# nickirk/pymes

Hardware: AMD Instinct MI355X
Metric: ccsd_iteration_time (lower is better)
Workload: dtype f64

## Files before the change

pymes_amd/csrc/kernels.hip:

```cpp
#include <hip/hip_runtime.h>
#include <type_traits>

#include <algorithm>
#include <atomic>
#include <chrono>
#include <cmath>
#include <cstdio>
#include <cstdlib>
#include <cstring>
#include <mutex>
#include <stdexcept>
#include <string>
#include <vector>

#include "device_api.h"
#include "diis_small.h"

#define HIP_CHECK(expr)                                                                   \
    do {                                                                                  \
        hipError_t err__ = (expr);                                                        \
        if (err__ != hipSuccess)                                                          \
            throw std::runtime_error(std::string("HIP error: ") + hipGetErrorString(err__) + \
                                     " at " __FILE__ ":" + std::to_string(__LINE__));     \
    } while (0)
// ... 1784 lines not shown
    const double* __restrict__ Ba = B + (long)(no + a) * n + no;
    const double* __restrict__ Bb = B + (long)(no + b) * n + no;
    const int t = threadIdx.x, lane = t & 63, w = t >> 6;
    const int wc = (w >> 1) * 16, wd = (w & 1) * 16, l15 = lane & 15, l4 = lane >> 4;
    const int lx = t & 31, lk = t >> 5;
    v4d X = {0.0, 0.0, 0.0, 0.0}, Y = {0.0, 0.0, 0.0, 0.0};
    for (int q0 = 0; q0 < naux; q0 += kFacK) {
#pragma unroll
        for (int h = 0; h < 2; ++h) {
            const int k = lk + 8 * h, q = q0 + k;
            const long qo = (long)q * nn;
            const bool cok = q < naux && c0 + lx < nv, dok = q < naux && d0 + lx < nv;
            sAc[k][lx] = cok ? Ba[qo + c0 + lx] : 0.0;
            sBc[k][lx] = cok ? Bb[qo + c0 + lx] : 0.0;
            sAd[k][lx] = dok ? Ba[qo + d0 + lx] : 0.0;
            sBd[k][lx] = dok ? Bb[qo + d0 + lx] : 0.0;
        }
        __syncthreads();
#pragma unroll
        for (int kk = 0; kk < kFacK; kk += 4) {
            const int k = kk + l4;
            X = __builtin_amdgcn_mfma_f64_16x16x4f64(sAc[k][wc + l15], sBd[k][wd + l15], X, 0, 0, 0);
            Y = __builtin_amdgcn_mfma_f64_16x16x4f64(sBc[k][wc + l15], sAd[k][wd + l15], Y, 0, 0, 0);
        }
        __syncthreads();
    }
    const int d = d0 + wd + l15;
#pragma unroll
    for (int i = 0; i < 4; ++i) {
        const int c = c0 + wc + l4 + 4 * i;
        if (c < nv && d < nv && c >= d) {
            Vp[row * npp + (long)c * (c + 1) / 2 + d] = X[i] + Y[i];
            if (c > d) Vm[row * npm + (long)c * (c - 1) / 2 + d] = (a > b) ? X[i] - Y[i] : 0.0;
        }
    }
}

__global__ void ladder_dress_tfrag_kernel(const double* __restrict__ t1, double* __restrict__ tf, int no, int nv, int nk, long total) {
    const long e = blockIdx.x * (long)blockDim.x + threadIdx.x;
    if (e >= total) return;
    const int L = (int)(e & 63), kk = (int)((e >> 6) % nk), tile = (int)((e >> 6) / nk);
    const int a = 16 * tile + (L & 15), k = 4 * kk + (L >> 4);
    tf[e] = (a < nv && k < no) ? -t1[(long)a * no + k] : 0.0;
}

template <int NK>
__global__ void __launch_bounds__(64) ladder_dress_kernel(const double* __restrict__ V, const double* __restrict__ Pk,
                                                          const double* __restrict__ tf, double* __restrict__ W, int no,
                                                          int nv, long ld, long row0, long row1, double sgn, long ntp) {
    constexpr int TP = 16 * 16 + 16;
    __shared__ double turn[16 * TP];
    const int lane = threadIdx.x, g = lane >> 4, c = lane & 15;
    const long idx = blockIdx.x >> 3;
    const long cdb = (blockIdx.x & 7) + 8 * (idx / ntp), tp = idx % ntp;
    if (cdb * 16 >= ld) return;
    int ta_, tb_;
    unrank_pair(tp, ta_, tb_);
    const int a0 = ta_ * 16, b0 = tb_ * 16;
    const long tri0 = (long)a0 * (a0 + 1) / 2;
    if (tri0 + (long)15 * a0 + 120 + b0 + 15 < row0 || tri0 + b0 >= row1) return;
    double ta[NK], tb[NK];
#pragma unroll
    for (int kk = 0; kk < NK; ++kk) {
        ta[kk] = tf[((long)ta_ * NK + kk) * 64 + lane];
        tb[kk] = tf[((long)tb_ * NK + kk) * 64 + lane];
    }
    typedef unsigned v2u __attribute__((ext_vector_type(2)));
    constexpr unsigned kOff = 0x80000000u;
    const long col = cdb * 16 + c;
    const unsigned lo = (unsigned)(8 * ((long)g * ld + col));
    const unsigned lo_last = (unsigned)(8 * ((long)(min(4 * (NK - 1) + g, no - 1) - 4 * (NK - 1)) * ld + col));
    const unsigned ldb = (unsigned)(8 * ld);
    const __amdgpu_buffer_rsrc_t rPa = __builtin_amdgcn_make_buffer_rsrc(const_cast<double*>(Pk + (long)a0 * no * ld), 0, kOff, 0x00020000);
    const __amdgpu_buffer_rsrc_t rPb = __builtin_amdgcn_make_buffer_rsrc(const_cast<double*>(Pk + (long)b0 * no * ld), 0, kOff, 0x00020000);
    const __amdgpu_buffer_rsrc_t rV = __builtin_amdgcn_make_buffer_rsrc(const_cast<double*>(V + (tri0 - row0) * ld), 0, kOff, 0x00020000);
    const __amdgpu_buffer_rsrc_t rW = __builtin_amdgcn_make_buffer_rsrc(W + (tri0 - row0) * ld, 0, kOff, 0x00020000);
    unsigned vo[4];
#pragma unroll
    for (int r = 0; r < 4; ++r) {
        const long a = a0 + g + 4 * r;
        vo[r] = a < nv ? (unsigned)(8 * ((a * (a + 1) / 2 - tri0) * ld + col)) : kOff;
    }
    auto row_off = [&](int r, int x) {
        const int a = a0 + g + 4 * r;
        const long row = (long)a * (a + 1) / 2 + x;
        return (x <= a && row >= row0 && row < row1) ? vo[r] : kOff;
    };
    constexpr int PA = 1, NBP = 2 * (PA + 1), VA = 3, NBV = 2 * (VA + 1);
    double pf[NBP][NK], vin[NBV][4];
    auto fetch_p = [&](int n) {
        const int x0 = n < 16 ? a0 : b0, i = n < 16 ? n : n - 16;
        const unsigned so = (unsigned)(min(x0 + i, nv - 1) - x0) * (unsigned)no * ldb;
        const __amdgpu_buffer_rsrc_t rs = n < 16 ? rPa : rPb;
#pragma unroll
        for (int kk = 0; kk < NK - 1; ++kk)
            pf[n % NBP][kk] = __builtin_bit_cast(double, __builtin_amdgcn_raw_buffer_load_b64(rs, lo, so + 4u * kk * ldb, 0));
        pf[n % NBP][NK - 1] = __builtin_bit_cast(double, __builtin_amdgcn_raw_buffer_load_b64(rs, lo_last, so + 4u * (NK - 1) * ldb, 0));
    };
    auto fetch_v = [&](int n) {
        const int x = b0 + n - 16;
#pragma unroll
        for (int r = 0; r < 4; ++r)
            vin[n % NBV][r] = __builtin_bit_cast(double, __builtin_amdgcn_raw_buffer_load_b64(rV, row_off(r, x), (unsigned)x * ldb, 2));
    };
#pragma unroll
    for (int n = 0; n < 2 * PA; ++n) fetch_p(n);
#pragma unroll
    for (int p = 0; p < 8; ++p) {
        const int n0 = 2 * p, n1 = n0 + 1;
        fetch_p(n0 + 2 * PA);
        fetch_p(n1 + 2 * PA);
        if (n0 + 2 * VA >= 16) { fetch_v(n0 + 2 * VA); fetch_v(n1 + 2 * VA); }
        v4d acc0 = {0.0, 0.0, 0.0, 0.0}, acc1 = {0.0, 0.0, 0.0, 0.0};
#pragma unroll
        for (int kk = 0; kk < NK; ++kk) {
            acc0 = __builtin_amdgcn_mfma_f64_16x16x4f64(tb[kk], pf[n0 % NBP][kk], acc0, 0, 0, 0);
            acc1 = __builtin_amdgcn_mfma_f64_16x16x4f64(tb[kk], pf[n1 % NBP][kk], acc1, 0, 0, 0);
        }
#pragma unroll
        for (int rb = 0; rb < 4; ++rb) {
            turn[n0 * TP + (g + 4 * rb) * 16 + c] = acc0[rb];
            turn[n1 * TP + (g + 4 * rb) * 16 + c] = acc1[rb];
        }
    }
    __builtin_amdgcn_fence(__ATOMIC_SEQ_CST, "wavefront");
    __builtin_amdgcn_wave_barrier();
    const double s2 = sgn > 0.0 ? -1.0 : 1.0;
#pragma unroll
    for (int p = 0; p < 8; ++p) {
        const int b = 2 * p, n0 = 16 + b, n1 = n0 + 1;
        if (n0 + 2 * PA < 32) { fetch_p(n0 + 2 * PA); fetch_p(n1 + 2 * PA); }
        if (n0 + 2 * VA < 32) { fetch_v(n0 + 2 * VA); fetch_v(n1 + 2 * VA); }
        v4d acc0, acc1;
#pragma unroll
        for (int r = 0; r < 4; ++r) {
            acc0[r] = fma(s2, turn[(g + 4 * r) * TP + b * 16 + c], vin[n0 % NBV][r]);
            acc1[r] = fma(s2, turn[(g + 4 * r) * TP + (b + 1) * 16 + c], vin[n1 % NBV][r]);
        }
#pragma unroll
        for (int kk = 0; kk < NK; ++kk) {
            acc0 = __builtin_amdgcn_mfma_f64_16x16x4f64(ta[kk], pf[n0 % NBP][kk], acc0, 0, 0, 0);
            acc1 = __builtin_amdgcn_mfma_f64_16x16x4f64(ta[kk], pf[n1 % NBP][kk], acc1, 0, 0, 0);
        }
#pragma unroll
        for (int h = 0; h < 2; ++h) {
            const int bb = b0 + b + h;
#pragma unroll
            for (int r = 0; r < 4; ++r) {
                const double val = (sgn > 0.0 && a0 + g + 4 * r == bb) ? 0.0 : (double)(h ? acc1[r] : acc0[r]);
                __builtin_amdgcn_raw_buffer_store_b64(__builtin_bit_cast(v2u, val), rW, row_off(r, bb), (unsigned)bb * ldb, 2);
            }
        }
    }
}

struct PackTK {
    const double* T; const double* t1; double* Sp; double* Am;
    long ldp, ldm, rp0;
    int no, nv, flags;
};
__device__ __forceinline__ void ladder_pack_T_body(const PackTK& k, const unsigned vb) {
    const double* __restrict__ T = k.T;
    const double* __restrict__ t1 = k.t1;
    double* __restrict__ Sp = k.Sp;
    double* __restrict__ Am = k.Am;
    const int no = k.no, nv = k.nv, flags = k.flags;
    const long ldp = k.ldp, ldm = k.ldm;
    const long row = k.rp0 + vb;
    int c, d;
    unrank_pair(row, c, d);
    const bool row_half = flags & dev::PACK_ROW_HALF, prow = flags & dev::PACK_AM_PROWS,
               col_half = flags & dev::PACK_COL_HALF, pcol = flags & dev::PACK_AM_PCOLS;
    const long o2 = (long)no * no;
    const double* __restrict__ T1 = T ? T + ((long)c * nv + d) * o2 : nullptr;
    const double* __restrict__ T2 = T ? T + ((long)d * nv + c) * o2 : nullptr;
    const double fr = (c == d && row_half) ? 0.25 : 0.5;
    const long mrow = prow ? row : (long)c * (c - 1) / 2 + d;
    const bool has_m = prow || c > d;
    if (threadIdx.x == 0) {
        const long opp = (long)no * (no + 1) / 2, mcols = pcol ? opp : opp - no;
        if (ldp > opp) Sp[row * ldp + opp] = 0.0;
        if (has_m && ldm > mcols) Am[mrow * ldm + mcols] = 0.0;
    }
    for (int e = threadIdx.x; e < o2; e += blockDim.x) {
        const int i = e / no, j = e - i * no;
        if (i < j) continue;
        double x1 = 0.0, x2 = 0.0;
        if (T) { x1 = T1[e]; x2 = T2[e]; }
        if (t1) {
            x1 += t1[(long)c * no + i] * t1[(long)d * no + j];
            x2 += t1[(long)d * no + i] * t1[(long)c * no + j];
        }
        Sp[row * ldp + (long)i * (i + 1) / 2 + j] = ((i == j && col_half) ? 0.5 * fr : fr) * (x1 + x2);
        if (has_m && (pcol || i > j)) {
            const long mcol = pcol ? (long)i * (i + 1) / 2 + j : (long)i * (i - 1) / 2 + j;
            Am[mrow * ldm + mcol] = (c > d && i > j) ? 0.5 * (x1 - x2) : 0.0;
        }
    }
}
__global__ void ladder_pack_T_kernel(const PackTK k) { ladder_pack_T_body(k, blockIdx.x); }

struct UnpackK {
    const double* L; double* R;
    double beta;
    long total;
    int no, nv;
};
__device__ __forceinline__ void ladder_unpack_body(const UnpackK& k, const unsigned vb, const unsigned vgrid) {
    const double* __restrict__ L = k.L;
    double* __restrict__ R = k.R;
    const double beta = k.beta;
    const int no = k.no, nv = k.nv;
    const long total = k.total;
    const long opp = (long)no * (no + 1) / 2, ld = (long)no * no;
    for (long idx = vb * (long)blockDim.x + threadIdx.x; idx < total; idx += (long)vgrid * blockDim.x) {
        long r = idx;
        const int j = (int)(r % no); r /= no;
        const int i = (int)(r % no); r /= no;
        const int b = (int)(r % nv);
        const int a = (int)(r / nv);
        const int ah = max(a, b), al = min(a, b), ih = max(i, j), il = min(i, j);
        const double* __restrict__ row = L + ((long)ah * (ah + 1) / 2 + al) * ld;
        double v = row[(long)ih * (ih + 1) / 2 + il];
        if (a != b && i != j) {
            const double x = row[opp + (long)ih * (ih - 1) / 2 + il];
            v += ((a > b) == (i > j)) ? x : -x;
        }
        R[idx] = (beta != 0.0) ? beta * R[idx] + v : v;
    }
}
__global__ void ladder_unpack_kernel(const UnpackK k) { ladder_unpack_body(k, blockIdx.x, gridDim.x); }

struct RingOpK {
    const double* Wd; const double* Ud; double* M; double* N1;
    double a1, a2;
    int no, nv;
};
__device__ __forceinline__ void ring_operands_body(const RingOpK& q, const unsigned vb) {
    const double* __restrict__ Wd = q.Wd;
    const double* __restrict__ Ud = q.Ud;
    double* __restrict__ M = q.M;
    double* __restrict__ N1 = q.N1;
    const double a1 = q.a1, a2 = q.a2;
    const int no = q.no, nv = q.nv;
    extern __shared__ double tile[];
    constexpr int CT = 32;
    const int k = vb / nv, b = vb - k * nv;
    const long ov = (long)no * nv;
    const double* __restrict__ wd = Wd + ((long)k * nv + b) * ((long)nv * no);
    const double* __restrict__ ud = Ud + ((long)k * nv + b) * ((long)no * nv);
    const long col = (long)b * no;
    for (int c0 = 0; c0 < nv; c0 += CT) {
        const int nc = min(CT, nv - c0);
        for (int e = threadIdx.x; e < no * CT; e += blockDim.x) {
            const int j = e / CT, cc = e - j * CT;
            if (cc < nc) tile[j * (CT + 1) + cc] = ud[(long)j * nv + c0 + cc];
        }
        __syncthreads();
        for (int e = threadIdx.x; e < nc * no; e += blockDim.x) {
            const int cc = e / no, j = e - cc * no;
            const double u = tile[j * (CT + 1) + cc];
            const double w = wd[(long)(c0 + cc) * no + j];
            const long off = ((long)(c0 + cc) * no + k) * ov + col + j;
            N1[off] = -u;
            M[off] = a1 * w - a2 * u;
        }
        __syncthreads();
    }
}
__global__ void __launch_bounds__(256) ring_operands_kernel(const RingOpK q) { ring_operands_body(q, blockIdx.x); }

struct LayoutsK {
    const double* T; double* Td; double* Tx; double* Ttd;
    double ca, cb;
    int no, nv;
};
template <bool RESIDUAL>
__device__ __forceinline__ void t2_layouts_body(const LayoutsK& k, const unsigned vb) {
    const double* __restrict__ T = k.T;
    double* __restrict__ Td = k.Td;
    double* __restrict__ Tx = k.Tx;
    double* __restrict__ Ttd = k.Ttd;
    const int no = k.no, nv = k.nv;
    const double ca = k.ca, cb = k.cb;
    extern __shared__ double tile[];
    const int a = vb / nv, b = vb - a * nv;
    const long o2 = (long)no * no, ov = (long)no * nv;
    const double* __restrict__ Tab = T + ((long)a * nv + b) * o2;
    const double* __restrict__ Tba = T + ((long)b * nv + a) * o2;
    const long base = (long)a * no * ov + (long)b * no;
    for (int e = threadIdx.x; e < o2; e += blockDim.x) {
        const int i = e / no, j = e - i * no;
        const double x = Tab[e];
        tile[i * (no + 1) + j] = x;
        const long off = base + (long)i * ov + j;
        if (Td) Td[off] = x;
        Ttd[off] = RESIDUAL ? 2.0 * x - Tba[e] : ca * x + cb * Tba[e];
    }
    __syncthreads();
    for (int e = threadIdx.x; e < o2; e += blockDim.x) {
        const int j = e / no, i = e - j * no;
        Tx[base + (long)j * ov + i] = tile[i * (no + 1) + j];
    }
}
template <bool RESIDUAL>
__global__ void __launch_bounds__(256) t2_layouts_kernel(const LayoutsK k) { t2_layouts_body<RESIDUAL>(k, blockIdx.x); }
// ... 2567 lines not shown
    };
    for (int i0 = 0; i0 < mx; i0 += 16)
        for (int j0 = 0; j0 < ny; j0 += 4) {
            const int mm = std::min(16, mx - i0), nn = std::min(4, ny - j0);
            int NN = 4;
            double* tile = tiles + 64 * done.size();
            if (mm <= 4) gram_tile_n<4>(X + i0, mm, Y + j0, nn, (long)len, vec, nblk, ws, tile, st, NN);
            else if (mm <= 8) gram_tile_n<8>(X + i0, mm, Y + j0, nn, (long)len, vec, nblk, ws, tile, st, NN);
            else if (mm <= 12) gram_tile_n<12>(X + i0, mm, Y + j0, nn, (long)len, vec, nblk, ws, tile, st, NN);
            else gram_tile_n<16>(X + i0, mm, Y + j0, nn, (long)len, vec, nblk, ws, tile, st, NN);
            done.push_back({i0, mm, j0, nn, NN});
            if ((int)done.size() == kGramTiles) flush();
        }
    flush();
}

void lincomb_multi(int m, int n, const double* const* x, const double* c, const double* beta, double* const* y, int64_t len,
                   stream_t s) {
    if (n <= 0 || len <= 0) return;
    if (m < 0 || m > 64 || n > 64) throw std::runtime_error("lincomb_multi: at most 64 inputs and 64 outputs per call");
    if (m > 16 || n > 4)
        for (int j = 0; j < n; ++j)
            for (int i = 0; i < m; ++i)
                if (y[j] == x[i]) throw std::runtime_error("lincomb_multi: an output may alias an input only for m <= 16, n <= 4");
    hipStream_t st = (hipStream_t)s;
    bool vec = true;
    for (int i = 0; i < m; ++i) vec = vec && aligned16(x[i]);
    for (int j = 0; j < n; ++j) vec = vec && aligned16(y[j]);
    double one[4] = {1.0, 1.0, 1.0, 1.0}, b0[4];
    for (int j0 = 0; j0 < n; j0 += 4) {
        const int nn = std::min(4, n - j0);
        for (int j = 0; j < nn; ++j) b0[j] = beta ? beta[j0 + j] : 0.0;
        if (m == 0) {
            const double* none[1] = {y[j0]};
            const double zero[4] = {0.0, 0.0, 0.0, 0.0};
            lincomb_multi_tile_n<4>(none, 1, zero, 4, b0, y + j0, nn, (long)len, vec, st);
            continue;
        }
        for (int i0 = 0; i0 < m; i0 += 16) {
            const int mm = std::min(16, m - i0);
            const double* bb = i0 == 0 ? b0 : one;
            const double* cc = c + (long)i0 * n + j0;
            if (mm <= 4) lincomb_multi_tile_n<4>(x + i0, mm, cc, n, bb, y + j0, nn, (long)len, vec, st);
            else if (mm <= 8) lincomb_multi_tile_n<8>(x + i0, mm, cc, n, bb, y + j0, nn, (long)len, vec, st);
            else if (mm <= 12) lincomb_multi_tile_n<12>(x + i0, mm, cc, n, bb, y + j0, nn, (long)len, vec, st);
            else lincomb_multi_tile_n<16>(x + i0, mm, cc, n, bb, y + j0, nn, (long)len, vec, st);
        }
    }
}

void cmul(const double* mr, const double* mi, const double* xr, const double* xi, double* yr, double* yi, int64_t n, stream_t s) {
    if (n <= 0) return;
    PYMES_LAUNCH(cmul_kernel, dim3(grid_for(n)), dim3(256), 0, (hipStream_t)s, mr, mi, xr, xi, yr, yi, (long)n);
    HIP_CHECK(hipGetLastError());
}

void exchange_split(const double* u, double* us, double* w, double* dg, int no, int nv, stream_t s) {
    const long total = (long)nv * nv * no * no;
    if (!total) return;
    PYMES_LAUNCH(exchange_split_kernel, dim3(grid_for(total, 256, 256 * 64)), dim3(256), 0, (hipStream_t)s, u, us, w, dg, no, nv,
                       total);
    HIP_CHECK(hipGetLastError());
}
void sgn_ij_add(double* D, const double* R, int no, int nv, stream_t s) {
    const long total = (long)nv * nv * no * no;
    if (!total) return;
    PYMES_LAUNCH(sgn_ij_add_kernel, dim3(grid_for(total, 256, 256 * 64)), dim3(256), 0, (hipStream_t)s, D, R, no, total);
    HIP_CHECK(hipGetLastError());
}
int64_t eom_diag_ws_doubles(int no, int nv) { return EomDiagWs(no, nv).total; }
void eom_diagonals(const double* V, const double* T, const double* dai, const double* iaai, const double* iaia, const double* ijij,
                   const double* abab, double* d1, double* d2, int no, int nv, double* ws, stream_t s) {
    hipStream_t st = (hipStream_t)s;
    const EomDiagWs w(no, nv);
    const long total = (long)nv * nv * no * no;
    if (w.total > 0x7fffffffL) throw std::runtime_error("eom_diagonals: problem too large for one grid");
    PYMES_LAUNCH(eom_diag_sums_kernel, dim3((unsigned)w.total), dim3(256), 0, st, V, T, ws, no, nv);
    HIP_CHECK(hipGetLastError());
    PYMES_LAUNCH(eom_diag_singles_kernel, dim3((unsigned)(((long)nv * no + 255) / 256)), dim3(256), 0, st, ws, dai, iaai, iaia,
                       d1, no, nv);
    HIP_CHECK(hipGetLastError());
    PYMES_LAUNCH(eom_diag_doubles_kernel, dim3(grid_for(total, 256, 256 * 64)), dim3(256), 0, st, V, T, ws, dai, iaai, iaia, ijij,
                       abab, d2, no, nv, total);
    HIP_CHECK(hipGetLastError());
}
void cshift_inv(const double* d, double zr, double zi, double hr, double hi, double shift, double* mr, double* mi, int64_t n,
                stream_t s) {
    if (n <= 0) return;
    PYMES_LAUNCH(cshift_inv_kernel, dim3(grid_for(n)), dim3(256), 0, (hipStream_t)s, d, zr, zi, hr, hi, shift, mr, mi, (long)n);
    HIP_CHECK(hipGetLastError());
}

void tau_build(double* tau, const double* t2, const double* t1, int no, int nv, stream_t s) {
    const long total = (long)nv * nv * no * no;
    if (!total) return;
    const TauK k{tau, t2, t1, total, no, nv};
    const double cost = 16.0 * (double)total / 4.0e6;
    if (phase_open((hipStream_t)s) && phase_small(cost)) {
        PhaseRec& t = phase_push(PK_TAU, 0, grid_for(total), 0, cost, k);
        phase_reads(t, {prange(t2, total), prange(t1, (long)no * nv)});
        phase_writes(t, {prange(tau, total)});
        return;
    }
    PYMES_LAUNCH(tau_kernel, dim3(grid_for(total)), dim3(256), 0, (hipStream_t)s, k);
    HIP_CHECK(hipGetLastError());
}

void ladder_pack_V(const double* V, double* Vp, double* Vm, int nr, int nc, int64_t rp0, int64_t rp1, stream_t s, int64_t ldvp,
                   int64_t ldvm) {
    if (rp1 <= rp0) return;
    const long npp = ldvp ? (long)ldvp : (long)nc * (nc + 1) / 2, npm = ldvm ? (long)ldvm : (long)nc * (nc - 1) / 2;
    const int nt = (nc + 31) / 32;
    const long ntp = (long)nt * (nt + 1) / 2;
    const long nblk = (rp1 - rp0) * ntp;
    if (nblk > 0x7fffffffL) throw std::runtime_error("ladder_pack_V: grid too large");
    PYMES_LAUNCH(ladder_pack_V_kernel, dim3((unsigned)nblk), dim3(256), 0, (hipStream_t)s, V, Vp, Vm, nr, nc,
                       (long)rp0, nt, ntp, npp, npm);
    HIP_CHECK(hipGetLastError());
}

void ladder_pack_V_factors(const double* B, double* Vp, double* Vm, int naux, int n, int no, int64_t rp0, int64_t rp1,
                           stream_t s, int64_t ldvp, int64_t ldvm) {
    if (rp1 <= rp0) return;
    const int nv = n - no;
    if (naux < 1 || no < 0 || nv < 1 || rp0 < 0 || rp1 > (int64_t)nv * (nv + 1) / 2)
        throw std::runtime_error("ladder_pack_V_factors: bad shape or pair-row range");
    const long npp = ldvp ? (long)ldvp : (long)nv * (nv + 1) / 2, npm = ldvm ? (long)ldvm : (long)nv * (nv - 1) / 2;
    const int nt = (nv + 31) / 32;
    const long ntp = (long)nt * (nt + 1) / 2;
    const long nblk = (rp1 - rp0) * ntp;
    if (nblk > 0x7fffffffL) throw std::runtime_error("ladder_pack_V_factors: grid too large");
    PYMES_LAUNCH(ladder_pack_V_factors_kernel, dim3((unsigned)nblk), dim3(256), 0, (hipStream_t)s, B, Vp, Vm, naux, n, no,
                 (long)rp0, ntp, npp, npm);
    HIP_CHECK(hipGetLastError());
}

bool ladder_dress_ok(int no, int nv) {
    const double ld = (double)((((long)nv * (nv + 1) / 2) + 15) & ~15L);
    return no >= 1 && no <= 80 && nv >= 1 && 8.0 * ld * (15.0 * nv + 137.0) < 2147483648.0;
}

int64_t ladder_dress_ws_doubles(int no, int nv) { return (int64_t)((nv + 15) / 16) * ((no + 3) / 4) * 64; }

void ladder_dress(const double* V, const double* Pk, const double* t1, double* W, int no, int nv, int64_t ld, int64_t row0,
                  int64_t row1, double sgn, double* ws, stream_t s) {
    if (!ladder_dress_ok(no, nv)) throw std::runtime_error("ladder_dress: nocc outside 1..80 or tile extents beyond 2 GB");
    if (ld <= 0 || (ld & 15)) throw std::runtime_error("ladder_dress: the row pitch must be a multiple of 16 doubles");
    if ((reinterpret_cast<uintptr_t>(V) | reinterpret_cast<uintptr_t>(Pk) | reinterpret_cast<uintptr_t>(W)) & 127)
        throw std::runtime_error("ladder_dress: operands must be 128-byte aligned");
    if (!ws) throw std::runtime_error("ladder_dress: workspace missing");
    const long npp = (long)nv * (nv + 1) / 2;
    if (row0 < 0 || row1 > npp || row0 > row1) throw std::runtime_error("ladder_dress: bad pair-row range");
    if (row1 == row0) return;
    const long nt = (nv + 15) / 16, ntp = nt * (nt + 1) / 2, ncdb = ld / 16, nblk = 8 * ((ncdb + 7) / 8) * ntp;
    if (nblk > 0x7fffffffL) throw std::runtime_error("ladder_dress: grid too large");
    if (8.0 * (double)ld * (15.0 * nv + 137.0) >= 2147483648.0) throw std::runtime_error("ladder_dress: tile extent exceeds the 2-GB buffer window");
    const dim3 grid((unsigned)nblk), block(64);
    hipStream_t st = (hipStream_t)s;
    const int nk = (no + 3) / 4;
    const long nfrag = ladder_dress_ws_doubles(no, nv);
    PYMES_LAUNCH(ladder_dress_tfrag_kernel, dim3((unsigned)((nfrag + 255) / 256)), dim3(256), 0, st, t1, ws, no, nv, nk, nfrag);
#define PYMES_DRESS(NK) case NK: PYMES_LAUNCH(ladder_dress_kernel<NK>, grid, block, 0, st, V, Pk, (const double*)ws, W, no, nv, (long)ld, (long)row0, (long)row1, sgn, ntp); break;
    switch (nk) {
        PYMES_DRESS(1) PYMES_DRESS(2) PYMES_DRESS(3) PYMES_DRESS(4) PYMES_DRESS(5) PYMES_DRESS(6) PYMES_DRESS(7) PYMES_DRESS(8)
        PYMES_DRESS(9) PYMES_DRESS(10) PYMES_DRESS(11) PYMES_DRESS(12) PYMES_DRESS(13) PYMES_DRESS(14) PYMES_DRESS(15) PYMES_DRESS(16)
        PYMES_DRESS(17) PYMES_DRESS(18) PYMES_DRESS(19) PYMES_DRESS(20)
    }
#undef PYMES_DRESS
    HIP_CHECK(hipGetLastError());
}

void ladder_pack_T(const double* X, const double* t1, double* Sp, double* Am, int nc, int nr, int flags, int64_t ldp,
                   int64_t ldm, stream_t s, int64_t rp0, int64_t rp1) {
    const long npp = (long)nr * (nr + 1) / 2, opp = (long)nc * (nc + 1) / 2, opm = (long)nc * (nc - 1) / 2;
    if (!ldp) ldp = opp;
    if (!ldm) ldm = (flags & PACK_AM_PCOLS) ? opp : opm;
    if (!X && !t1) throw std::runtime_error("ladder_pack_T: nothing to pack");
    if (rp1 < 0) { rp0 = 0; rp1 = npp; }
    if (rp0 < 0 || rp1 > npp || rp0 > rp1) throw std::runtime_error("ladder_pack_T: bad row range");
    if ((rp0 != 0 || rp1 != npp) && !(flags & PACK_AM_PROWS)) throw std::runtime_error("ladder_pack_T: a row range needs PACK_AM_PROWS");
    if (rp1 == rp0) return;
    const PackTK k{X, t1, Sp, Am, (long)ldp, (long)ldm, (long)rp0, nc, nr, flags};
    const double cost = 24.0 * (double)(rp1 - rp0) * (double)nc * (double)nc / 4.0e6;
    if (phase_open((hipStream_t)s) && phase_small(cost)) {
        PhaseRec& t = phase_push(PK_PACK_T, 0, rp1 - rp0, 0, cost, k);
        phase_reads(t, {prange(X, X ? (long)nr * nr * nc * nc : 0), prange(t1, t1 ? (long)nr * nc : 0)});
        const long am_rows = (flags & PACK_AM_PROWS) ? npp : (long)nr * (nr - 1) / 2;
        phase_writes(t, {pbox(Sp + rp0 * ldp, {{rp1 - rp0, ldp}, {ldp, 1}}),
                         (flags & PACK_AM_PROWS) ? pbox(Am + rp0 * ldm, {{rp1 - rp0, ldm}, {ldm, 1}}) : prange(Am, am_rows * ldm)});
        return;
    }
    PYMES_LAUNCH(ladder_pack_T_kernel, dim3((unsigned)(rp1 - rp0)), dim3(256), 0, (hipStream_t)s, k);
    HIP_CHECK(hipGetLastError());
}

void ladder_unpack(const double* L, double* R, double beta, int no, int nv, stream_t s) {
    const long total = (long)nv * nv * no * no;
    if (!total) return;
    const UnpackK k{L, R, beta, total, no, nv};
    const double cost = 20.0 * (double)total / 4.0e6;
    if (phase_open((hipStream_t)s) && phase_small(cost)) {
        PhaseRec& t = phase_push(PK_LADDER_UNPACK, 0, grid_for(total), 0, cost, k);
        phase_reads(t, {prange(L, (long)nv * (nv + 1) / 2 * no * no)});
        phase_writes(t, {prange(R, total)});
        return;
    }
    PYMES_LAUNCH(ladder_unpack_kernel, dim3(grid_for(total)), dim3(256), 0, (hipStream_t)s, k);
    HIP_CHECK(hipGetLastError());
}

bool fused_pair_kernels_ok(int no) { return (size_t)no * (no + 1) * sizeof(double) <= 64 * 1024; }

void ring_operands(const double* Viabj, const double* Viajb, double* M, double* N1, double a1, double a2, int no, int nv,
                   stream_t s) {
    if (no < 1 || nv < 1) return;
    const size_t lds = sizeof(double) * (size_t)no * 33;
    if (lds > 64 * 1024) throw std::runtime_error("ring_operands: nocc too large for the LDS tile");
    const RingOpK k{Viabj, Viajb, M, N1, a1, a2, no, nv};
    const long ov2 = (long)no * nv * no * nv;
    const double cost = 32.0 * (double)ov2 / 4.0e6;
    if (phase_open((hipStream_t)s) && phase_small(cost)) {
        PhaseRec& t = phase_push(PK_RING_OPERANDS, 0, (long)no * nv, (int)lds, cost, k);
        phase_reads(t, {prange(Viabj, ov2), prange(Viajb, ov2)});
        phase_writes(t, {prange(M, ov2), prange(N1, ov2)});
        return;
    }
    PYMES_LAUNCH(ring_operands_kernel, dim3((unsigned)((long)no * nv)), dim3(256), lds, (hipStream_t)s, k);
    HIP_CHECK(hipGetLastError());
}

void t2_layouts(const double* T, double* Td, double* Tx, double* Ttd, int no, int nv, stream_t s, double ca, double cb) {
    if (!fused_pair_kernels_ok(no)) throw std::runtime_error("t2_layouts: nocc too large for the LDS tile");
    const size_t lds = sizeof(double) * no * (no + 1);
    const LayoutsK k{T, Td, Tx, Ttd, ca, cb, no, nv};
    const bool res = ca == 2.0 && cb == -1.0;
    const long n4 = (long)nv * nv * no * no;
    const double cost = 40.0 * (double)n4 / 4.0e6;
    if (phase_open((hipStream_t)s) && phase_small(cost)) {
        PhaseRec& t = phase_push(PK_T2_LAYOUTS, res ? 1 : 0, (long)nv * nv, (int)lds, cost, k);
        phase_reads(t, {prange(T, n4)});
        phase_writes(t, {prange(Td, Td ? n4 : 0), prange(Tx, n4), prange(Ttd, n4)});
        return;
    }
    if (res) PYMES_LAUNCH(t2_layouts_kernel<true>, dim3((unsigned)(nv * nv)), dim3(256), lds, (hipStream_t)s, k);
    else PYMES_LAUNCH(t2_layouts_kernel<false>, dim3((unsigned)(nv * nv)), dim3(256), lds, (hipStream_t)s, k);
    HIP_CHECK(hipGetLastError());
}

void residual_assemble(const double* V, const double* L, const double* N, const double* D, const double* X, double* R,
                       int no, int nv, stream_t s, double xd) {
    if (!fused_pair_kernels_ok(no)) throw std::runtime_error("residual_assemble: nocc too large for the LDS tile");
    const size_t lds = sizeof(double) * no * (no + 1);
    const AssembleK k{V, L, N, D, X, R, xd, no, nv};
    const long n4 = (long)nv * nv * no * no;
    const double cost = 48.0 * (double)n4 / 4.0e6;
    if (phase_open((hipStream_t)s) && phase_small(cost)) {
        PhaseRec& t = phase_push(PK_ASSEMBLE, 0, (long)nv * (nv + 1) / 2, (int)lds, cost, k);
        phase_reads(t, {prange(V, V ? n4 : 0), prange(L, L ? (long)nv * (nv + 1) / 2 * no * no : 0), prange(N, n4), prange(D, n4), prange(X, n4)});
        phase_writes(t, {prange(R, n4)});
        return;
    }
    PYMES_LAUNCH(residual_assemble_kernel, dim3((unsigned)((long)nv * (nv + 1) / 2)), dim3(256), lds, (hipStream_t)s, k);
    HIP_CHECK(hipGetLastError());
}

void scatter(double* dst, const int64_t* idx_host, const double* val_host, int64_t n, stream_t s) {
    if (n <= 0) return;
    long* idx = nullptr;
    double* val = nullptr;
    HIP_CHECK(hipMalloc(&idx, sizeof(long) * n));
    if (hipMalloc(&val, sizeof(double) * n) != hipSuccess) { (void)hipFree(idx); throw std::runtime_error("scatter: out of device memory"); }
    hipStream_t st = (hipStream_t)s;
    HIP_CHECK(hipMemcpyAsync(idx, idx_host, sizeof(long) * n, hipMemcpyHostToDevice, st));
    HIP_CHECK(hipMemcpyAsync(val, val_host, sizeof(double) * n, hipMemcpyHostToDevice, st));
    PYMES_LAUNCH(scatter_kernel, dim3(grid_for(n)), dim3(256), 0, st, dst, idx, val, (long)n);
    const hipError_t e = hipGetLastError();
    (void)hipStreamSynchronize(st);
    (void)hipFree(idx);
    (void)hipFree(val);
    HIP_CHECK(e);
}

void hf_fock(const double* const dir[4], const double* const exc[4], const double* h_dev, double* f_dev, int no, int nv,
             stream_t s) {
    HfBlocks B;
    for (int i = 0; i < 4; ++i) { B.dir[i] = dir[i]; B.exc[i] = exc[i]; }
    const int n = no + nv;
    PYMES_LAUNCH(hf_fock_kernel, dim3((n * n + 255) / 256), dim3(256), 0, (hipStream_t)s, B, h_dev, f_dev, no, nv);
    HIP_CHECK(hipGetLastError());
}

int64_t fcidump_fill(double* V, const double* val_host, const int32_t* pqrs_host, int64_t count, int n, bool is_tc,
                     stream_t s) {
    if (count <= 0) return 0;
    hipStream_t st = (hipStream_t)s;
    const int64_t chunk = 1 << 22;
    double* dval = nullptr;
    int* didx = nullptr;
    unsigned long long* dbad = nullptr;
    unsigned long long bad = 0;
    HIP_CHECK(hipMalloc(&dval, sizeof(double) * std::min(count, chunk)));
    if (hipMalloc(&didx, sizeof(int) * 4 * std::min(count, chunk)) != hipSuccess || hipMalloc(&dbad, sizeof(bad)) != hipSuccess) {
        (void)hipFree(dval); (void)hipFree(didx);
        throw std::runtime_error("fcidump_fill: out of device memory");
    }
    hipError_t err = hipMemsetAsync(dbad, 0, sizeof(bad), st);
    for (int pass = 0; pass < 2 && err == hipSuccess; ++pass)
        for (int64_t b0 = 0; b0 < count && err == hipSuccess; b0 += chunk) {
            const int64_t nb = std::min(chunk, count - b0);
            err = hipMemcpyAsync(dval, val_host + b0, sizeof(double) * nb, hipMemcpyHostToDevice, st);
            if (err == hipSuccess) err = hipMemcpyAsync(didx, pqrs_host + 4 * b0, sizeof(int) * 4 * nb, hipMemcpyHostToDevice, st);
            if (err != hipSuccess) break;
            PYMES_LAUNCH(fcidump_fill_kernel, dim3(grid_for(nb)), dim3(256), 0, st, V, dval, didx, (long)nb, (long)n,
                               is_tc ? 1 : 0, pass, dbad);
            err = hipGetLastError();
            if (err == hipSuccess) err = hipStreamSynchronize(st);
        }
    if (err == hipSuccess) err = hipMemcpy(&bad, dbad, sizeof(bad), hipMemcpyDeviceToHost);
    (void)hipFree(dval); (void)hipFree(didx); (void)hipFree(dbad);
    HIP_CHECK(err);
    return (int64_t)bad;
// ... 615 lines not shown
```

Baseline: 0.1638.

## Add wide 32-column ladder dress kernel with LDS transpose for small nocc

Adds a new ladder_dress variant in which each 64-lane block covers 32 columns using 128-bit buffer loads and stores and two MFMA accumulators per row. The t1 contraction over both pair indices is reordered to go through an LDS turnaround buffer, and there are separate edge and interior template paths. The goal is to halve the number of blocks, widen memory transactions, and give each t1 fragment load more reuse. The cost is higher register pressure from the hold and pf buffers and the LDS allocation, which may lower occupancy for larger NK. The launcher picks this kernel whenever nocc/4 is 15 or less.

```diff
diff --git a/pymes_amd/csrc/kernels.hip b/pymes_amd/csrc/kernels.hip
--- a/pymes_amd/csrc/kernels.hip
+++ b/pymes_amd/csrc/kernels.hip
@@ -1960,6 +1960,154 @@
             }
         }
     }
+}
+
+constexpr int kDressWideNK = 15;
+template <int NK, bool EDGE>
+__device__ __forceinline__ void ladder_dress_wide_body(const double* __restrict__ V, const double* __restrict__ Pk,
+                                                       const double* __restrict__ tf, double* __restrict__ W, int no, int nv,
+                                                       long ld, long row0, long row1, double sgn, int ta_, int tb_, long cdb,
+                                                       double* __restrict__ turn) {
+    typedef unsigned v4u __attribute__((ext_vector_type(4)));
+    typedef double v2d __attribute__((ext_vector_type(2)));
+    const int lane = threadIdx.x, g = lane >> 4, c = lane & 15;
+    const int a0 = ta_ * 16, b0 = tb_ * 16;
+    const long tri0 = (long)a0 * (a0 + 1) / 2;
+    const double s2 = sgn > 0.0 ? -1.0 : 1.0;
+    double ta[NK], tb[NK];
+#pragma unroll
+    for (int kk = 0; kk < NK; ++kk) {
+        ta[kk] = tf[((long)ta_ * NK + kk) * 64 + lane];
+        tb[kk] = s2 * tf[((long)tb_ * NK + kk) * 64 + lane];
+    }
+    constexpr unsigned kOff = 0x80000000u;
+    const long col = cdb * 32 + 2 * c;
+    const bool colok = col < ld;
+    const unsigned ldb = (unsigned)(8 * ld);
+    const unsigned lo = colok ? (unsigned)(8 * ((long)g * ld + col)) : kOff;
+    const unsigned lo_last = colok ? (unsigned)(8 * ((long)(min(4 * (NK - 1) + g, no - 1) - 4 * (NK - 1)) * ld + col)) : kOff;
+    const __amdgpu_buffer_rsrc_t rPa = __builtin_amdgcn_make_buffer_rsrc(const_cast<double*>(Pk + (long)a0 * no * ld), 0, kOff, 0x00020000);
+    const __amdgpu_buffer_rsrc_t rPb = __builtin_amdgcn_make_buffer_rsrc(const_cast<double*>(Pk + (long)b0 * no * ld), 0, kOff, 0x00020000);
+    const __amdgpu_buffer_rsrc_t rV = __builtin_amdgcn_make_buffer_rsrc(const_cast<double*>(V + (tri0 - row0) * ld), 0, kOff, 0x00020000);
+    const __amdgpu_buffer_rsrc_t rW = __builtin_amdgcn_make_buffer_rsrc(W + (tri0 - row0) * ld, 0, kOff, 0x00020000);
+    unsigned vb[4], vo[4];
+#pragma unroll
+    for (int r = 0; r < 4; ++r) {
+        const long a = a0 + g + 4 * r;
+        vb[r] = colok ? (unsigned)(8 * ((long)(g + 4 * r) * ld + col)) : kOff;
+        vo[r] = colok ? (unsigned)(8 * ((a * (a + 1) / 2 - tri0) * ld + col)) : kOff;
+    }
+    auto row_ok = [&](int a, int b) {
+        const long row = (long)a * (a + 1) / 2 + b;
+        return a < nv && b <= a && row >= row0 && row < row1;
+    };
+    constexpr int PA = NK <= 13 ? 2 : 1, NBP = PA + 1, VA = 3, NBV = VA + 1;
+    v2d pf[NBP][NK], vin[NBV][4], hold[16][2];
+    auto fetch_p = [&](int n) {
+        const int x0 = n < 16 ? a0 : b0, i = n < 16 ? n : n - 16;
+        const unsigned so = (unsigned)(min(x0 + i, nv - 1) - x0) * (unsigned)no * ldb;
+        const __amdgpu_buffer_rsrc_t rs = n < 16 ? rPa : rPb;
+#pragma unroll
+        for (int kk = 0; kk < NK - 1; ++kk)
+            pf[n % NBP][kk] = __builtin_bit_cast(v2d, __builtin_amdgcn_raw_buffer_load_b128(rs, lo, so + 4u * kk * ldb, 0));
+        pf[n % NBP][NK - 1] = __builtin_bit_cast(v2d, __builtin_amdgcn_raw_buffer_load_b128(rs, lo_last, so + 4u * (NK - 1) * ldb, 0));
+    };
+    auto fetch_v = [&](int n) {
+        const int a = a0 + n;
+        const unsigned so = (unsigned)((long)a * (a + 1) / 2 - tri0 + b0) * ldb;
+#pragma unroll
+        for (int r = 0; r < 4; ++r) {
+            const unsigned off = (!EDGE || row_ok(a, b0 + g + 4 * r)) ? vb[r] : kOff;
+            vin[n % NBV][r] = __builtin_bit_cast(v2d, __builtin_amdgcn_raw_buffer_load_b128(rV, off, so, 2));
+        }
+    };
+    auto turn_write = [&](int n, v2d lo_b, v2d hi_b) {
+        *reinterpret_cast<v2d*>(turn + (n * 8 + g) * 32 + 2 * c) = lo_b;
+        *reinterpret_cast<v2d*>(turn + (n * 8 + g + 4) * 32 + 2 * c) = hi_b;
+    };
+    auto wave_sync = [&]() {
+        __builtin_amdgcn_fence(__ATOMIC_SEQ_CST, "wavefront");
+        __builtin_amdgcn_wave_barrier();
+    };
+#pragma unroll
+    for (int n = 0; n < PA; ++n) fetch_p(n);
+#pragma unroll
+    for (int n = 0; n < VA; ++n) fetch_v(n);
+#pragma unroll
+    for (int n = 0; n < 16; ++n) {
+        fetch_p(n + PA);
+        if (n + VA < 16) fetch_v(n + VA);
+        v4d acc0, acc1;
+#pragma unroll
+        for (int r = 0; r < 4; ++r) {
+            acc0[r] = vin[n % NBV][r][0];
+            acc1[r] = vin[n % NBV][r][1];
+        }
+#pragma unroll
+        for (int kk = 0; kk < NK; ++kk) {
+            acc0 = __builtin_amdgcn_mfma_f64_16x16x4f64(tb[kk], pf[n % NBP][kk][0], acc0, 0, 0, 0);
+            acc1 = __builtin_amdgcn_mfma_f64_16x16x4f64(tb[kk], pf[n % NBP][kk][1], acc1, 0, 0, 0);
+        }
+        turn_write(n, v2d{acc0[0], acc1[0]}, v2d{acc0[1], acc1[1]});
+        hold[n][0] = v2d{acc0[2], acc1[2]};
+        hold[n][1] = v2d{acc0[3], acc1[3]};
+    }
+#pragma unroll
+    for (int h = 0; h < 2; ++h) {
+        if (h == 1) {
+            wave_sync();
+#pragma unroll
+            for (int n = 0; n < 16; ++n) turn_write(n, hold[n][0], hold[n][1]);
+        }
+        wave_sync();
+#pragma unroll
+        for (int j = 0; j < 8; ++j) {
+            const int b = 8 * h + j, n = 16 + b, bb = b0 + b;
+            if (n + PA < 32) fetch_p(n + PA);
+            v4d acc0, acc1;
+#pragma unroll
+            for (int r = 0; r < 4; ++r) {
+                const v2d d2 = *reinterpret_cast<const v2d*>(turn + ((g + 4 * r) * 8 + j) * 32 + 2 * c);
+                acc0[r] = d2[0];
+                acc1[r] = d2[1];
+            }
+#pragma unroll
+            for (int kk = 0; kk < NK; ++kk) {
+                acc0 = __builtin_amdgcn_mfma_f64_16x16x4f64(ta[kk], pf[n % NBP][kk][0], acc0, 0, 0, 0);
+                acc1 = __builtin_amdgcn_mfma_f64_16x16x4f64(ta[kk], pf[n % NBP][kk][1], acc1, 0, 0, 0);
+            }
+#pragma unroll
+            for (int r = 0; r < 4; ++r) {
+                const int a = a0 + g + 4 * r;
+                v2d val = {acc0[r], acc1[r]};
+                unsigned off = vo[r];
+                if (EDGE) {
+                    if (sgn > 0.0 && a == bb) val = v2d{0.0, 0.0};
+                    if (!row_ok(a, bb)) off = kOff;
+                }
+                __builtin_amdgcn_raw_buffer_store_b128(__builtin_bit_cast(v4u, val), rW, off, (unsigned)bb * ldb, 2);
+            }
+        }
+    }
+}
+
+template <int NK>
+__global__ void __launch_bounds__(64) ladder_dress_wide_kernel(const double* __restrict__ V, const double* __restrict__ Pk,
+                                                               const double* __restrict__ tf, double* __restrict__ W, int no,
+                                                               int nv, long ld, long row0, long row1, double sgn, long ntp) {
+    __shared__ __attribute__((aligned(16))) double turn[16 * 8 * 32];
+    const long idx = blockIdx.x >> 3;
+    const long cdb = (blockIdx.x & 7) + 8 * (idx / ntp), tp = idx % ntp;
+    if (cdb * 32 >= ld) return;
+    int ta_, tb_;
+    unrank_pair(tp, ta_, tb_);
+    const int a0 = ta_ * 16, b0 = tb_ * 16;
+    const long first = (long)a0 * (a0 + 1) / 2 + b0, last = first + (long)15 * a0 + 135;
+    if (last < row0 || first >= row1) return;
+    if (a0 == b0 || a0 + 15 >= nv || first < row0 || last >= row1)
+        ladder_dress_wide_body<NK, true>(V, Pk, tf, W, no, nv, ld, row0, row1, sgn, ta_, tb_, cdb, turn);
+    else
+        ladder_dress_wide_body<NK, false>(V, Pk, tf, W, no, nv, ld, row0, row1, sgn, ta_, tb_, cdb, turn);
 }
 
 struct PackTK {
@@ -4833,21 +4981,27 @@
     const long npp = (long)nv * (nv + 1) / 2;
     if (row0 < 0 || row1 > npp || row0 > row1) throw std::runtime_error("ladder_dress: bad pair-row range");
     if (row1 == row0) return;
-    const long nt = (nv + 15) / 16, ntp = nt * (nt + 1) / 2, ncdb = ld / 16, nblk = 8 * ((ncdb + 7) / 8) * ntp;
+    const int nk = (no + 3) / 4;
+    const bool wide = nk <= kDressWideNK;
+    const long nt = (nv + 15) / 16, ntp = nt * (nt + 1) / 2, ncdb = wide ? (ld + 31) / 32 : ld / 16, nblk = 8 * ((ncdb + 7) / 8) * ntp;
     if (nblk > 0x7fffffffL) throw std::runtime_error("ladder_dress: grid too large");
     if (8.0 * (double)ld * (15.0 * nv + 137.0) >= 2147483648.0) throw std::runtime_error("ladder_dress: tile extent exceeds the 2-GB buffer window");
     const dim3 grid((unsigned)nblk), block(64);
     hipStream_t st = (hipStream_t)s;
-    const int nk = (no + 3) / 4;
     const long nfrag = ladder_dress_ws_doubles(no, nv);
     PYMES_LAUNCH(ladder_dress_tfrag_kernel, dim3((unsigned)((nfrag + 255) / 256)), dim3(256), 0, st, t1, ws, no, nv, nk, nfrag);
-#define PYMES_DRESS(NK) case NK: PYMES_LAUNCH(ladder_dress_kernel<NK>, grid, block, 0, st, V, Pk, (const double*)ws, W, no, nv, (long)ld, (long)row0, (long)row1, sgn, ntp); break;
+#define PYMES_DRESS_ARGS grid, block, 0, st, V, Pk, (const double*)ws, W, no, nv, (long)ld, (long)row0, (long)row1, sgn, ntp
+#define PYMES_DRESS_WIDE(NK) case NK: PYMES_LAUNCH(ladder_dress_wide_kernel<NK>, PYMES_DRESS_ARGS); break;
+#define PYMES_DRESS(NK) case NK: PYMES_LAUNCH(ladder_dress_kernel<NK>, PYMES_DRESS_ARGS); break;
     switch (nk) {
-        PYMES_DRESS(1) PYMES_DRESS(2) PYMES_DRESS(3) PYMES_DRESS(4) PYMES_DRESS(5) PYMES_DRESS(6) PYMES_DRESS(7) PYMES_DRESS(8)
-        PYMES_DRESS(9) PYMES_DRESS(10) PYMES_DRESS(11) PYMES_DRESS(12) PYMES_DRESS(13) PYMES_DRESS(14) PYMES_DRESS(15) PYMES_DRESS(16)
+        PYMES_DRESS_WIDE(1) PYMES_DRESS_WIDE(2) PYMES_DRESS_WIDE(3) PYMES_DRESS_WIDE(4) PYMES_DRESS_WIDE(5) PYMES_DRESS_WIDE(6)
+        PYMES_DRESS_WIDE(7) PYMES_DRESS_WIDE(8) PYMES_DRESS_WIDE(9) PYMES_DRESS_WIDE(10) PYMES_DRESS_WIDE(11) PYMES_DRESS_WIDE(12)
+        PYMES_DRESS_WIDE(13) PYMES_DRESS_WIDE(14) PYMES_DRESS_WIDE(15) PYMES_DRESS(16)
         PYMES_DRESS(17) PYMES_DRESS(18) PYMES_DRESS(19) PYMES_DRESS(20)
     }
 #undef PYMES_DRESS
+#undef PYMES_DRESS_WIDE
+#undef PYMES_DRESS_ARGS
     HIP_CHECK(hipGetLastError());
 }
 
```

New measurement: 0.1628 (median of 6 runs). Within noise of the previous version (-0.6%).
